# nomadoor/ComfyUI-Video-Stabilizer

Hardware: AMD Instinct MI355X
Metric: stabilized frames/sec (1080p, similarity mode) (higher is better)
Workload: dtype f32; 1 GPU; C2: 256-frame clip, 1920x1080, Video Stabilizer Flow (DIS) similarity + crop_and_pad, defaults (strength 0.7, smooth 0.5, 16 fps), device-resident in/out, entered at the node's input adaptation; frames_per_gpu=256, total_frames=256

## Files before the change

### comfyui-video-stabilizer_amd/csrc/vstab_dis.hip

```cpp
#include "vstab_internal.h"
#include <cstdlib>
#include <cfloat>
#include <algorithm>
#include <cmath>
#include <memory>

namespace {

constexpr float DIS_EPS = 0.001f;
constexpr float DIS_INF = 1e10f;
constexpr int DIS_BORDER = 16;
constexpr int PSZ = 8;
constexpr int PSTR = 4;
constexpr int DEFAULT_FINEST = 2;
constexpr int GD_ITERS = 25;
constexpr int VAR_ITERS = 5;
constexpr int SOR_ITERS = 5;
constexpr int MAX_LEVELS = 16;

struct LevelGeom {
    int w, h, ws, hs;
};

unsigned grid_for(long long items, int block = 256)
// ... 141 lines not shown
        const AreaTaps& ax = s_x[x];
        const AreaTaps& ay = s_y[ry];
        float sum = 0.f;
        for (int j = 0; j < ay.n; j++) {
            const uint8_t* row = S + (size_t)(ay.first + j) * sw + ax.first;
            float buf = 0.f;
            for (int k = 0; k < ax.n; k++) buf += row[k] * ax.a[k];
            const float term = ay.a[j] * buf;
            sum = (j == 0) ? term : sum + term;
        }
        D[t] = (uint8_t)sat_u8_round(sum);
    }
}

constexpr int TAIL_MAX_LEVELS = 8;
#ifdef VSTAB_FUSED_TRACE
#define TAIL_MARK(i) do { if (prof_) { const long long now_ = wall_clock64(); a.dbg[i] += now_ - tprev_; tprev_ = now_; } } while (0)
#else
#define TAIL_MARK(i)
#endif
struct TailLevel { uint8_t* dst; int h, w, mode, kx, ky; double scale_x, scale_y; };
struct TailArgs {
#ifdef VSTAB_FUSED_TRACE
    long long* dbg;
#endif
    const uint8_t* src;
    int n, h0, w0, levels;
    TailLevel lv[TAIL_MAX_LEVELS];
    uint8_t* prep_ext;
    short* prep_ix;
    short* prep_iy;
    float* prep_tensor;
    int prep_ws, prep_hs, prep_lds_off;
};

__global__ __launch_bounds__(1024) void pyramid_tail_kernel(TailArgs a)
{
    extern __shared__ __attribute__((aligned(16))) unsigned char tail_lds[];
    const int f = blockIdx.x;
#ifdef VSTAB_FUSED_TRACE
    long long tprev_ = wall_clock64();
    const bool prof_ = a.dbg && blockIdx.x == 7 && threadIdx.x == 0;
#endif
    const int cap0 = (a.h0 * a.w0 + 15) & ~15;
    const int cap1 = (a.lv[0].h * a.lv[0].w + 15) & ~15;
    unsigned char* bufA = tail_lds;
    unsigned char* bufB = tail_lds + cap0;
    AreaTaps* s_x = reinterpret_cast<AreaTaps*>(tail_lds + cap0 + cap1);
    AreaTaps* s_y = s_x + a.lv[0].w;
    {
        const uint8_t* S = a.src + (size_t)f * a.h0 * a.w0;
        const int npx = a.h0 * a.w0;
        if ((reinterpret_cast<uintptr_t>(S) & 3) == 0 && (npx & 3) == 0) {
            const unsigned* s4 = reinterpret_cast<const unsigned*>(S);
            unsigned* d4 = reinterpret_cast<unsigned*>(bufA);
            for (int k = threadIdx.x; k < npx / 4; k += blockDim.x) d4[k] = s4[k];
        } else {
            for (int k = threadIdx.x; k < npx; k += blockDim.x) bufA[k] = S[k];
        }
    }
    __syncthreads();
    TAIL_MARK(0);
    int sh = a.h0, sw = a.w0;
    unsigned char* cur = bufA;
    unsigned char* nxt = bufB;
    for (int l = 0; l < a.levels; l++) {
        const TailLevel& L = a.lv[l];
        const int dh = L.h, dw = L.w;
        if (L.mode == 2) {
            for (int x = threadIdx.x; x < dw; x += blockDim.x) area_taps(x, sw, L.scale_x, s_x[x]);
            for (int y = threadIdx.x; y < dh; y += blockDim.x) area_taps(y, sh, L.scale_y, s_y[y]);
            __syncthreads();
        }
        uint8_t* D = L.dst + (size_t)f * dh * dw;
        if (L.mode == 2 && L.kx <= 4 && L.ky <= 4 && dw <= (int)blockDim.x) {
            const int rows_par = (int)blockDim.x / dw;
            const int x = (int)threadIdx.x % dw, ry = (int)threadIdx.x / dw;
            if (ry < rows_par) {
                const AreaTaps ax = s_x[x];
                const int x0 = ax.first;
                for (int y = ry; y < dh; y += rows_par) {
                    const AreaTaps& ay = s_y[y];
// ... 1122 lines not shown
            Ixs[i] = c.take<short>(px);
            Iys[i] = c.take<short>(px);
            tensor[i] = c.take<float>(5 * (size_t)n * G[i].hs * G[i].ws);
            Ul[i] = c.take<float>((size_t)P * G[i].h * G[i].w);
            Vl[i] = c.take<float>((size_t)P * G[i].h * G[i].w);
        }
        aux = c.take<float>(5 * (size_t)n * F.h * F.ws);
        aux_c = c.take<float>(5 * (size_t)n * G[coarsest].h * G[coarsest].ws);
        Sx = c.take<float>((size_t)P * F.hs * F.ws);
        Sy = c.take<float>((size_t)P * F.hs * F.ws);
        vb.avg = c.take<float>(npF); vb.Iz = c.take<float>(npF);
        vb.D0 = c.take<f4_t>(npF); vb.D1 = c.take<f4_t>(npF);
        vb.UV = c.take<f2_t>(npF); vb.dA = c.take<f2_t>(npF); vb.dB = c.take<f2_t>(npF);
    };
    {
        Carver sizer(nullptr);
        layout(sizer);
        if (ctx->d_dis.reserve(sizer.off + 256)) return 1;
    }
    Carver carver(ctx->d_dis.ptr);
    layout(carver);

    static const bool two_streams = [] { const char* e = getenv("VSTAB_DIS_PREP_STREAM"); return !(e && atoi(e) == 0); }();
    static_assert(sizeof(ctx->ev_prep) / sizeof(ctx->ev_prep[0]) >= MAX_LEVELS, "one event per pyramid level");
    hipStream_t ps = st;
    if (two_streams) {
        VSTAB_HIP(ctx->prep_stream.ensure());
        VSTAB_HIP(ctx->ev_pyramid.ensure());
        for (auto& ev : ctx->ev_prep) VSTAB_HIP(ev.ensure());
        ps = ctx->prep_stream;
    }
    auto prep_timer = std::make_unique<KernelTimer>(ctx, "dis_prep", KernelTimer::DETAIL);
    bool coarsest_prepared = false;
    {
        if (launch_area(st, gray, I[FINEST], n, h, w, G[FINEST].h, G[FINEST].w)) return 1;
        static const bool tail_on = [] { const char* e = getenv("VSTAB_DIS_PYRAMID_TAIL"); return !(e && atoi(e) == 0); }();
        const int tail_levels = coarsest - FINEST;
        size_t tail_lds = 0;
        if (tail_levels >= 1) {
            const LevelGeom& a0 = G[FINEST];
            const LevelGeom& a1 = G[FINEST + 1];
            tail_lds = (((size_t)a0.h * a0.w + 15) & ~size_t(15)) + (((size_t)a1.h * a1.w + 15) & ~size_t(15)) +
                       sizeof(AreaTaps) * ((size_t)a1.w + a1.h);
        }
        if (tail_on && tail_levels >= 1 && tail_levels <= TAIL_MAX_LEVELS && tail_lds <= 150 * 1024) {
            TailArgs ta{};
#ifdef VSTAB_FUSED_TRACE
            ta.dbg = g_dis_dbg ? g_dis_dbg + 16 * 7 : nullptr;
#endif
            {
                const LevelGeom& c = G[coarsest];
                const size_t off = (tail_lds + 15) & ~size_t(15);
                const size_t need = (((size_t)4 * c.h * c.w + 15) & ~size_t(15)) + sizeof(float) * 5 * (size_t)c.h * c.ws;
                if (off + need <= 150 * 1024) {
                    ta.prep_ext = Iext[coarsest]; ta.prep_ix = Ixs[coarsest]; ta.prep_iy = Iys[coarsest]; ta.prep_tensor = tensor[coarsest];
                    ta.prep_ws = c.ws; ta.prep_hs = c.hs; ta.prep_lds_off = (int)off;
                    tail_lds = off + need;
                    coarsest_prepared = true;
                }
            }
            ta.src = I[FINEST]; ta.n = n; ta.h0 = G[FINEST].h; ta.w0 = G[FINEST].w; ta.levels = tail_levels;
            for (int i = FINEST + 1; i <= coarsest; i++) {
                AreaPlan pl;
                if (int rc = plan_area(G[i - 1].h, G[i - 1].w, G[i].h, G[i].w, pl)) return rc;
                TailLevel& tl = ta.lv[i - FINEST - 1];
                tl.dst = I[i]; tl.h = G[i].h; tl.w = G[i].w; tl.mode = pl.mode; tl.kx = pl.isx; tl.ky = pl.isy;
                if (pl.mode == 2) {
                    tl.kx = (int)std::floor(pl.scale_x) + 2; tl.ky = (int)std::floor(pl.scale_y) + 2;
                }
                tl.scale_x = pl.scale_x; tl.scale_y = pl.scale_y;
            }
            if (tail_lds > 64 * 1024)
                VSTAB_HIP(hipFuncSetAttribute(reinterpret_cast<const void*>(pyramid_tail_kernel), hipFuncAttributeMaxDynamicSharedMemorySize, (int)tail_lds));
            hipLaunchKernelGGL(pyramid_tail_kernel, dim3((unsigned)n), dim3(1024), tail_lds, st, ta);
            VSTAB_HIP(hipGetLastError());
        } else {
            for (int i = FINEST + 1; i <= coarsest; i++)
                if (launch_area(st, I[i - 1], I[i], n, G[i - 1].h, G[i - 1].w, G[i].h, G[i].w)) return 1;
        }
    }
    if (two_streams) {
        VSTAB_HIP(hipEventRecord(ctx->ev_pyramid, st));
        VSTAB_HIP(hipStreamWaitEvent(ps, ctx->ev_pyramid, 0));
    }
    for (int i = coarsest; i >= FINEST; i--) {
        const LevelGeom& g = G[i];
        const bool own = i == coarsest;
        if (own && coarsest_prepared) continue;
        hipStream_t s_i = own ? st : ps;
        float* aux_i = own ? aux_c : aux;
        hipLaunchKernelGGL(pad_replicate_kernel, frame_grid((long long)(g.h + 32) * (g.w + 32), n), dim3(256), 0, s_i, I[i], Iext[i], n, g.h, g.w);
        hipLaunchKernelGGL(sobel_kernel, frame_grid((long long)g.h * g.w, n), dim3(256), 0, s_i, I[i], Ixs[i], Iys[i], n, g.h, g.w);
        hipLaunchKernelGGL(tensor_h_kernel, frame_grid((long long)g.h * g.ws, n), dim3(256), 0, s_i, Ixs[i], Iys[i], aux_i, n, g.h, g.w, g.ws);
        hipLaunchKernelGGL(tensor_v_kernel, dim3((unsigned)((g.ws + 63) / 64), (unsigned)n, 5u), dim3(64), 0, s_i, aux_i, tensor[i], n, g.h, g.ws, g.hs);
        VSTAB_HIP(hipGetLastError());
        if (two_streams && !own) VSTAB_HIP(hipEventRecord(ctx->ev_prep[i], ps));
    }
    VSTAB_HIP(hipMemsetAsync(Ul[coarsest], 0, sizeof(float) * (size_t)P * G[coarsest].h * G[coarsest].w, st));
    VSTAB_HIP(hipMemsetAsync(Vl[coarsest], 0, sizeof(float) * (size_t)P * G[coarsest].h * G[coarsest].w, st));

    prep_timer.reset();

    bool grid_fused = false;
    const float zeta = 0.1f, epsilon = 0.001f, alpha = 20.0f, delta = 5.0f, gamma = 10.0f, omega = 1.6f;
    const float zeta2 = zeta * zeta, eps2 = epsilon * epsilon, gamma2 = gamma / 2, delta2 = delta / 2, alpha2 = alpha / 4;

    for (int i = coarsest; i >= FINEST; i--) {
        const LevelGeom& g = G[i];
        PisArgs pa{};
        pa.I = I[i]; pa.Iext = Iext[i]; pa.Ix = Ixs[i]; pa.Iy = Iys[i]; pa.tensor = tensor[i];
        pa.U = Ul[i]; pa.V = Vl[i]; pa.Sx = Sx; pa.Sy = Sy;
        pa.n = n; pa.w = g.w; pa.h = g.h; pa.ws = g.ws; pa.hs = g.hs;
        pa.stripe_sz = (int)std::ceil(g.hs / 8.0);
        pa.spin_limit = 1 << 22;
#ifdef VSTAB_TEST_HOOKS
        if (const char* e = getenv("VSTAB_DEBUG_PIS_SPIN_LIMIT")) pa.spin_limit = atoi(e);
#endif
        pa.status = ctx->status.dev<int>();
        if (two_streams && i != coarsest) VSTAB_HIP(hipStreamWaitEvent(st, ctx->ev_prep[i], 0));
        const size_t lds_bytes = (((size_t)(g.w + 32) * (g.h + 32) + 15) & ~size_t(15)) + sizeof(float) * 2 * (size_t)g.hs * g.ws + sizeof(int) * 2 * (size_t)g.hs;
        VSTAB_REQUIRE(lds_bytes <= 160 * 1024, "vstab_dis_flow_batch: level %dx%d needs %zu B of LDS (> 160 KB)", g.w, g.h, lds_bytes);
        char kind_pis[24], kind_level[24];
        snprintf(kind_pis, sizeof(kind_pis), "dis_pis4_L%d", i);
        snprintf(kind_level, sizeof(kind_level), "dis_level_L%d", i);
        auto stage_timer = std::make_unique<KernelTimer>(ctx, kind_pis, KernelTimer::DETAIL);
        if (pa.stripe_sz > 4) {
            if (lds_bytes > 64 * 1024)
                VSTAB_HIP(hipFuncSetAttribute(reinterpret_cast<const void*>(pis4_kernel<2>), hipFuncAttributeMaxDynamicSharedMemorySize, (int)lds_bytes));
            hipLaunchKernelGGL(pis4_kernel<2>, dim3((unsigned)P * 2), dim3(64 * 2 * PIS_STRIPES_PER_BLOCK), lds_bytes, st, pa);
        } else {
            if (lds_bytes > 64 * 1024)
                VSTAB_HIP(hipFuncSetAttribute(reinterpret_cast<const void*>(pis4_kernel<1>), hipFuncAttributeMaxDynamicSharedMemorySize, (int)lds_bytes));
// ... 118 lines not shown
```

### comfyui-video-stabilizer_amd/csrc/vstab_fit.hip

```cpp
#include "vstab_fit_common.h"

namespace {

#ifndef VSTAB_FIT_THREADS
#define VSTAB_FIT_THREADS 512
#endif
constexpr int FIT_THREADS = VSTAB_FIT_THREADS;
constexpr int FIT_WAVES = FIT_THREADS / 64;
static_assert(FIT_THREADS >= 256 && FIT_THREADS % 64 == 0 && FIT_THREADS <= 1024, "radix_select uses 256 histogram bins");
constexpr int RANSAC_BATCH = 16;
constexpr int MAX_SORT = 16384;

struct FitArgs {
    const float* grid_flow;
    int* vmap;
    vstab_fit_record* out;
    int pairs, gh, gw, step, requested_mode;
    const int* counts;
    int cap;
    const uint8_t* blocked;
};

__device__ void identity_record(vstab_fit_record& r, int nv, int total)
{
    for (int i = 0; i < 9; i++) r.matrix[i] = (i % 4 == 0) ? 1.f : 0.f;
    r.confidence = 0.0; r.residual = 0.0; r.accepted = 0; r.computed = 0; r.valid_points = nv; r.total_points = total;
}

__device__ __forceinline__ unsigned sort_key(float v)
{
    const unsigned b = __float_as_uint(v);
    return (b & 0x80000000u) ? ~b : (b | 0x80000000u);
}
__device__ __forceinline__ float key_value(unsigned k)
{
    return __uint_as_float((k & 0x80000000u) ? (k & 0x7fffffffu) : ~k);
}

__device__ unsigned radix_select(const unsigned* keys, int n, int r, int* hist , int* ctl )
{
    unsigned prefix = 0, mask = 0;
    for (int shift = 24; shift >= 0; shift -= 8) {
        if (threadIdx.x < 256) hist[threadIdx.x] = 0;
        __syncthreads();
        for (int k = threadIdx.x; k < n; k += FIT_THREADS) {
            const unsigned key = keys[k];
            if ((key & mask) == prefix) atomicAdd(&hist[(key >> shift) & 255u], 1);
        }
        __syncthreads();
        if (threadIdx.x < 64) {
            const int l = threadIdx.x;
            const int h0 = hist[4 * l], h1 = hist[4 * l + 1], h2 = hist[4 * l + 2], h3 = hist[4 * l + 3];
            const int mine = h0 + h1 + h2 + h3;
            int incl = mine;
#pragma unroll
            for (int d = 1; d < 64; d <<= 1) {
                const int o = __shfl_up(incl, d);
                if (l >= d) incl += o;
            }
            const int excl = incl - mine;
            if (r >= excl && r < incl) {
                int rr = r - excl, b = 4 * l;
                if (rr >= h0) { rr -= h0; b++; if (rr >= h1) { rr -= h1; b++; if (rr >= h2) { rr -= h2; b++; } } }
                ctl[0] = b; ctl[1] = rr;
            }
        }
        __syncthreads();
        prefix |= (unsigned)ctl[0] << shift;
        mask |= 0xffu << shift;
        r = ctl[1];
        __syncthreads();
    }
    return prefix;
}

template <bool MASKED>
__global__ __launch_bounds__(FIT_THREADS) void fit_kernel(FitArgs a)
{
    __shared__ unsigned s_sort[MAX_SORT];
    __shared__ int s_hist[256];
    __shared__ int s_sel[2];
    __shared__ double s_model[RANSAC_BATCH][6];
    __shared__ float s_modelf[RANSAC_BATCH][6];
    __shared__ int s_idx[RANSAC_BATCH][2];
    __shared__ int s_cnt[RANSAC_BATCH];
    __shared__ double s_red[FIT_WAVES];
    __shared__ int s_redi[FIT_WAVES];
    __shared__ int s_scan[FIT_THREADS];
    __shared__ double s_best[6];
    __shared__ int s_ctl[4];
    __shared__ Rng s_rng;

    const int pair = blockIdx.x, tid = threadIdx.x;
    const bool points = a.gw == 0;
    const int scan = points ? a.counts[pair] : a.gh * a.gw;
    const uint8_t* __restrict__ B0 = MASKED ? a.blocked + (size_t)pair * a.cap : nullptr;
    const uint8_t* __restrict__ B1 = MASKED ? B0 + a.cap : nullptr;
    int* __restrict__ vmap = a.vmap + (size_t)pair * a.cap;
    const Samples smp{a.grid_flow + (size_t)pair * a.cap * (points ? 4 : 2), vmap, a.gw, a.step};
    vstab_fit_record* out = a.out + (size_t)pair * 3;

    const int per = (scan + FIT_THREADS - 1) / FIT_THREADS;
    const int g0 = tid * per, g1 = min(g0 + per, scan);
    int local = 0, admitted = 0;
    for (int g = g0; g < g1; g++) {
        float px, py, cx, cy;
        smp.load(g, px, py, cx, cy);
        if (MASKED) {
            const bool adm = (B0[g] | B1[g]) == 0;
            admitted += adm ? 1 : 0;
            local += (adm && isfinite(cx) && isfinite(cy)) ? 1 : 0;
        } else {
            local += (isfinite(cx) && isfinite(cy)) ? 1 : 0;
        }
    }
    int total = scan;
    if (MASKED) total = block_sum<FIT_WAVES>(admitted, s_redi);
    {
        int incl = local;
#pragma unroll
        for (int d = 1; d < 64; d <<= 1) {
            const int o = __shfl_up(incl, d);
            if ((tid & 63) >= d) incl += o;
        }
        if ((tid & 63) == 63) s_redi[tid >> 6] = incl;
        __syncthreads();
        int before = 0;
        for (int i = 0; i < (tid >> 6); i++) before += s_redi[i];
        s_scan[tid] = before + incl - local;
        if (tid == FIT_THREADS - 1) s_sel[0] = before + incl;
    }
    __syncthreads();
    const int nv = s_sel[0];
    {
        int o = s_scan[tid];
        for (int g = g0; g < g1; g++) {
            float px, py, cx, cy;
            smp.load(g, px, py, cx, cy);
            if ((!MASKED || (B0[g] | B1[g]) == 0) && isfinite(cx) && isfinite(cy)) vmap[o++] = g;
        }
    }
    __syncthreads();
    if (tid < 3) identity_record(out[tid], nv, total);
    if (points ? (total < 12 || nv < 8) : nv < 12) return;
    __threadfence_block();
    __syncthreads();

    if (a.requested_mode >= VSTAB_MODE_SIMILARITY && nv >= 3) {
        if (tid == 0) { s_rng.state = ~0ULL; s_ctl[0] = 0; s_ctl[1] = 2000; s_ctl[2] = 0; s_ctl[3] = 0; }
        __syncthreads();
        const float thr = (float)(2.0 * 2.0);
        while (true) {
            if (tid == 0) {
                Rng r = s_rng;
                for (int c = 0; c < RANSAC_BATCH; c++) {
                    const int i0 = rng_uniform(r, 0, nv);
                    int i1;
                    do { i1 = rng_uniform(r, 0, nv); } while (i1 == i0);
                    s_idx[c][0] = i0; s_idx[c][1] = i1;
                }
                s_rng = r;
            }
            __syncthreads();
            if (tid < RANSAC_BATCH) {
                float x1f, y1f, X1f, Y1f, x2f, y2f, X2f, Y2f;
                smp.load(vmap[s_idx[tid][0]], x1f, y1f, X1f, Y1f);
                smp.load(vmap[s_idx[tid][1]], x2f, y2f, X2f, Y2f);
                const double x1 = x1f, y1 = y1f, x2 = x2f, y2 = y2f, X1 = X1f, Y1 = Y1f, X2 = X2f, Y2 = Y2f;
                const double d = 1. / ((x1 - x2) * (x1 - x2) + (y1 - y2) * (y1 - y2));
                const double S0 = d * ((X1 - X2) * (x1 - x2) + (Y1 - Y2) * (y1 - y2));
                const double S1 = d * ((Y1 - Y2) * (x1 - x2) - (X1 - X2) * (y1 - y2));
                const double S2 = d * ((Y1 - Y2) * (x1 * y2 - x2 * y1) - (X1 * y2 - X2 * y1) * (y1 - y2) - (X1 * x2 - X2 * x1) * (x1 - x2));
                const double S3 = d * (-(X1 - X2) * (x1 * y2 - x2 * y1) - (Y1 * x2 - Y2 * x1) * (x1 - x2) - (Y1 * y2 - Y2 * y1) * (y1 - y2));
                const double M[6] = {S0, -S1, S2, S1, S0, S3};
                for (int k = 0; k < 6; k++) { s_model[tid][k] = M[k]; s_modelf[tid][k] = (float)M[k]; }
                s_cnt[tid] = 0;
            }
            __syncthreads();
            ransac_score_batch<RANSAC_BATCH, FIT_THREADS>(smp, nv, thr, s_cnt, [&](int c, float px, float py, float cx, float cy) {
                return affine_err2(s_modelf[c], px, py, cx, cy);
            });
            __syncthreads();
            if (tid == 0) ransac_replay<RANSAC_BATCH, 6, 2, 1>(s_ctl, s_cnt, s_model, s_best, nv, [](int) { return RANSAC_SOLVED; });
            __syncthreads();
            if (s_ctl[0]) break;
        }
        const int maxGood = s_ctl[3];
        if (maxGood > 0) {
            const float Bf[6] = {(float)s_best[0], (float)s_best[1], (float)s_best[2], (float)s_best[3], (float)s_best[4], (float)s_best[5]};
            double sxx = 0, sx = 0, sy = 0, sX = 0, sY = 0, sxX = 0, syX = 0;
            int ninl = 0;
            smp.for_each_valid<FIT_THREADS>(nv, [&](int, float px, float py, float cx, float cy) {
                if (affine_err2(Bf, px, py, cx, cy) <= thr) {
                    const double x = px, y = py, X = cx, Y = cy;
                    sxx += x * x + y * y; sx += x; sy += y; sX += X; sY += Y;
                    sxX += x * X + y * Y; syX += x * Y - y * X;
                    ninl++;
                }
            });
            sxx = block_sum<FIT_WAVES>(sxx, s_red); sx = block_sum<FIT_WAVES>(sx, s_red); sy = block_sum<FIT_WAVES>(sy, s_red);
            sX = block_sum<FIT_WAVES>(sX, s_red); sY = block_sum<FIT_WAVES>(sY, s_red);
            sxX = block_sum<FIT_WAVES>(sxX, s_red); syX = block_sum<FIT_WAVES>(syX, s_red);
            ninl = block_sum<FIT_WAVES>(ninl, s_redi);
            if (tid == 0) {
                double A[4][5] = {{sxx, 0, sx, sy, sxX}, {0, sxx, -sy, sx, syX}, {sx, -sy, (double)ninl, 0, sX}, {sy, sx, 0, (double)ninl, sY}};
                bool ok = true;
                for (int col = 0; col < 4 && ok; col++) {
                    int piv = col;
                    for (int r = col + 1; r < 4; r++) if (fabs(A[r][col]) > fabs(A[piv][col])) piv = r;
                    if (fabs(A[piv][col]) < 1e-300) { ok = false; break; }
                    if (piv != col) for (int k = 0; k < 5; k++) { const double t = A[piv][k]; A[piv][k] = A[col][k]; A[col][k] = t; }
                    for (int r = col + 1; r < 4; r++) {
                        const double f = A[r][col] / A[col][col];
                        for (int k = col; k < 5; k++) A[r][k] -= f * A[col][k];
                    }
                }
                double sol[4] = {s_best[0], s_best[3], s_best[2], s_best[5]};
                if (ok && ninl > 0) {
                    for (int r = 3; r >= 0; r--) {
                        double v = A[r][4];
                        for (int k = r + 1; k < 4; k++) v -= A[r][k] * sol[k];
                        sol[r] = v / A[r][r];
                    }
                }
                s_best[0] = sol[0]; s_best[1] = -sol[1]; s_best[2] = sol[2];
                s_best[3] = sol[1]; s_best[4] = sol[0]; s_best[5] = sol[3];
            }
            __syncthreads();
            const double M0 = s_best[0], M1 = s_best[1], M2 = s_best[2], M3 = s_best[3], M4 = s_best[4], M5 = s_best[5];
            double res = 0;
            smp.for_each_valid<FIT_THREADS>(nv, [&](int, float px, float py, float cx, float cy) {
                const double x = px, y = py;
                res += fabs(x * M0 + y * M1 + M2 - (double)cx) + fabs(x * M3 + y * M4 + M5 - (double)cy);
            });
            res = block_sum<FIT_WAVES>(res, s_red);
            if (tid == 0) {
                vstab_fit_record& r = out[VSTAB_MODE_SIMILARITY];
                r.computed = 1;
                r.confidence = (double)maxGood / (double)nv;
                if (r.confidence >= 0.1) {
                    r.matrix[0] = (float)M0; r.matrix[1] = (float)M1; r.matrix[2] = (float)M2;
                    r.matrix[3] = (float)M3; r.matrix[4] = (float)M4; r.matrix[5] = (float)M5;
                    r.matrix[6] = 0.f; r.matrix[7] = 0.f; r.matrix[8] = 1.f;
                    r.residual = res / (2.0 * nv);
                    r.accepted = 1;
                }
            }
        } else if (tid == 0) {
            out[VSTAB_MODE_SIMILARITY].computed = 1;
        }
        __syncthreads();
    }

    {
        float med[2];
        for (int axis = 0; axis < 2; axis++) {
            smp.for_each_valid<FIT_THREADS>(nv, [&](int k, float px, float py, float cx, float cy) {
                s_sort[k] = sort_key(axis == 0 ? cx - px : cy - py);
            });
            __syncthreads();
            const int mid = nv / 2;
            const unsigned hi = radix_select(s_sort, nv, mid, s_hist, s_sel);
            if (nv & 1) {
                med[axis] = key_value(hi);
            } else {
                int less = 0;
                unsigned below = 0;
                for (int i = tid; i < nv; i += FIT_THREADS) {
                    const unsigned key = s_sort[i];
                    if (key < hi) { less++; below = key > below ? key : below; }
                }
#pragma unroll
                for (int sft = 32; sft > 0; sft >>= 1) {
                    less += __shfl_down(less, sft);
                    const unsigned o = __shfl_down(below, sft);
                    below = o > below ? o : below;
                }
                if ((tid & 63) == 0) { s_redi[tid >> 6] = less; s_hist[tid >> 6] = (int)below; }
                __syncthreads();
                int total_less = 0;
                unsigned mx = 0;
                for (int i = 0; i < FIT_WAVES; i++) { total_less += s_redi[i]; mx = (unsigned)s_hist[i] > mx ? (unsigned)s_hist[i] : mx; }
                const unsigned lo = total_less == mid ? mx : hi;
                med[axis] = (key_value(lo) + key_value(hi)) / 2.0f;
            }
            __syncthreads();
        }
        const float tx = med[0], ty = med[1];
        double res = 0;
        smp.for_each_valid<FIT_THREADS>(nv, [&](int, float px, float py, float cx, float cy) {
            res += (double)__builtin_fabsf((px + tx) - cx) + (double)__builtin_fabsf((py + ty) - cy);
        });
        res = block_sum<FIT_WAVES>(res, s_red);
        if (tid == 0) {
            vstab_fit_record& r = out[VSTAB_MODE_TRANSLATION];
            r.computed = 1; r.accepted = 1;
            r.matrix[2] = tx; r.matrix[5] = ty;
            r.confidence = (double)nv / (double)total;
            r.residual = res / (2.0 * nv);
        }
    }
}

}

int vstab_fit_homography(vstab_ctx* ctx, const float* grid_flow, const int* vmap, int pairs, int gh, int gw, int step,
                         int cap, vstab_fit_record* d_out);

static int run_fit(vstab_ctx* ctx, const float* data, const int* counts, int pairs, int gh, int gw, int step, int cap,
                   int requested_mode, vstab_fit_record* results, const uint8_t* blocked = nullptr)
{
    VSTAB_HIP(hipSetDevice(ctx->device));
    if (ctx->fit_pairs_pending > 0 && ctx->fit_copy_bytes == 0 && ctx->ev_fit_done) VSTAB_HIP(hipEventSynchronize(ctx->ev_fit_done));
    ctx->fit_pairs_pending = 0; ctx->fit_copy_bytes = 0;
    const size_t rec_bytes = sizeof(vstab_fit_record) * (size_t)pairs * 3;
    const size_t map_bytes = sizeof(int) * (size_t)pairs * cap;
    if (ctx->d_fit.reserve(rec_bytes + map_bytes + 512)) return 1;
    if (ctx->h_fit.reserve(rec_bytes)) return 1;
    char* base = static_cast<char*>(ctx->d_fit.ptr);
// ... 100 lines not shown
```

### comfyui-video-stabilizer_amd/csrc/vstab_fit_common.h

```cpp
#pragma once
#include "vstab_internal.h"
#include <cmath>

namespace {

struct Rng { unsigned long long state; };
__device__ __forceinline__ unsigned rng_next(Rng& r)
{
    r.state = (unsigned long long)(unsigned)r.state * 4164903690ULL + (unsigned)(r.state >> 32);
    return (unsigned)r.state;
}
__device__ __forceinline__ int rng_uniform(Rng& r, int a, int b) { return a == b ? a : (int)(rng_next(r) % (unsigned)(b - a) + a); }

__device__ int ransac_update_num_iters(double p, double ep, int modelPoints, int maxIters)
{
    p = p > 0. ? p : 0.; p = p < 1. ? p : 1.;
    ep = ep > 0. ? ep : 0.; ep = ep < 1. ? ep : 1.;
    double num = 1. - p > 2.2250738585072014e-308 ? 1. - p : 2.2250738585072014e-308;
    double denom = 1. - pow(1. - ep, (double)modelPoints);
    if (denom < 2.2250738585072014e-308) return 0;
    num = log(num);
    denom = log(denom);
    return denom >= 0 || -num >= maxIters * (-denom) ? maxIters : (int)__builtin_rint(num / denom);
}

struct Samples {
    const float* F;
    const int* vmap;
    int gw, step;

    __device__ __forceinline__ void load(int g, float& px, float& py, float& cx, float& cy) const
    {
        if (gw == 0) {
            const float4 v = *reinterpret_cast<const float4*>(F + (size_t)g * 4);
            px = v.x; py = v.y; cx = v.z; cy = v.w;
            return;
        }
        const int gy = g / gw, gx = g - gy * gw;
        px = (float)(gx * step);
        py = (float)(gy * step);
        cx = px + F[(size_t)g * 2];
        cy = py + F[(size_t)g * 2 + 1];
    }

    template <int NT, typename Body>
    __device__ __forceinline__ void for_each_valid(int nv, Body&& body) const
    {
        for (int k = threadIdx.x; k < nv; k += NT) {
            float px, py, cx, cy;
            load(vmap[k], px, py, cx, cy);
            body(k, px, py, cx, cy);
        }
    }
};

template <int WAVES, typename T>
__device__ __forceinline__ T block_sum(T v, T* scratch )
{
#pragma unroll
    for (int s = 32; s > 0; s >>= 1) v += __shfl_down(v, s);
    __syncthreads();
    if ((threadIdx.x & 63) == 0) scratch[threadIdx.x >> 6] = v;
    __syncthreads();
    T total = scratch[0];
#pragma unroll
    for (int i = 1; i < WAVES; i++) total += scratch[i];
    __syncthreads();
    return total;
}

__device__ __forceinline__ float affine_err2(const float* M, float px, float py, float cx, float cy)
{
    const float ea = M[0] * px + M[1] * py + M[2] - cx;
    const float eb = M[3] * px + M[4] * py + M[5] - cy;
    return ea * ea + eb * eb;
}
__device__ __forceinline__ float reproj_err2(const float* H, float px, float py, float cx, float cy)
{
    const float ww = 1.f / (H[6] * px + H[7] * py + 1.f);
    const float ex = (H[0] * px + H[1] * py + H[2]) * ww - cx;
    const float ey = (H[3] * px + H[4] * py + H[5]) * ww - cy;
    return ex * ex + ey * ey;
}

template <int BATCH, int NT, typename Err>
__device__ __forceinline__ void ransac_score_batch(const Samples& samples, int nv, float thr, int* s_cnt, Err&& err)
{
    int cnt[BATCH];
#pragma unroll
    for (int c = 0; c < BATCH; c++) cnt[c] = 0;
    samples.for_each_valid<NT>(nv, [&](int, float px, float py, float cx, float cy) {
#pragma unroll
        for (int c = 0; c < BATCH; c++) cnt[c] += (err(c, px, py, cx, cy) <= thr) ? 1 : 0;
    });
#pragma unroll
    for (int c = 0; c < BATCH; c++) {
        int v = cnt[c];
#pragma unroll
        for (int s = 32; s > 0; s >>= 1) v += __shfl_down(v, s);
        if ((threadIdx.x & 63) == 0 && v) atomicAdd(&s_cnt[c], v);
    }
// ... 26 lines not shown
```

### comfyui-video-stabilizer_amd/csrc/vstab_homography.hip

```cpp
#include "vstab_fit_common.h"

#define VSTAB_HAVE_HOMOGRAPHY 1

namespace {

constexpr int HT = 256;
constexpr int HBATCH = 16;
constexpr int HWAVES = HT / 64;

struct JacWs {
    double A[81];
    double V[81];
    double W[9];
    int indR[9], indC[9];
    double norm[8];
    int go, pad_;
    double pad;
};

__device__ __forceinline__ void group_sync()
{
    __builtin_amdgcn_fence(__ATOMIC_ACQ_REL, "wavefront");
    __builtin_amdgcn_wave_barrier();
}
// ... 146 lines not shown
            for (int k = j; k < 9; k++) LtL[j * 9 + k] += Lx[j] * Lx[k] + Ly[j] * Ly[k];
    }
    ws.norm[0] = cmx; ws.norm[1] = cmy; ws.norm[2] = cMx; ws.norm[3] = cMy;
    ws.norm[4] = smx; ws.norm[5] = smy; ws.norm[6] = sMx; ws.norm[7] = sMy;
    return true;
}

__device__ bool collinear(const float* p, int count)
{
    const int i = count - 1;
    for (int j = 0; j < i; j++) {
        double dx1 = p[j * 2] - p[i * 2], dy1 = p[j * 2 + 1] - p[i * 2 + 1];
        for (int k = 0; k < j; k++) {
            double dx2 = p[k * 2] - p[i * 2], dy2 = p[k * 2 + 1] - p[i * 2 + 1];
            if (fabs(dx2 * dy1 - dy2 * dx1) <= 1.1920928955078125e-07 * (fabs(dx1) + fabs(dy1) + fabs(dx2) + fabs(dy2))) return true;
        }
    }
    return false;
}
__device__ double det3pts(const float* p, int t0, int t1, int t2)
{
    const double a0 = p[t0 * 2], a1 = p[t0 * 2 + 1], a3 = p[t1 * 2], a4 = p[t1 * 2 + 1], a6 = p[t2 * 2], a7 = p[t2 * 2 + 1];
    return a0 * (a4 * 1. - 1. * a7) - a1 * (a3 * 1. - 1. * a6) + 1. * (a3 * a7 - a4 * a6);
}
__device__ bool check_subset(const float* ms1, const float* ms2)
{
    if (collinear(ms1, 4) || collinear(ms2, 4)) return false;
    const int tt[4][3] = {{0, 1, 2}, {1, 2, 3}, {0, 2, 3}, {0, 1, 3}};
    int negative = 0;
    for (int i = 0; i < 4; i++) negative += det3pts(ms1, tt[i][0], tt[i][1], tt[i][2]) * det3pts(ms2, tt[i][0], tt[i][1], tt[i][2]) < 0;
    return negative == 0 || negative == 4;
}

template <int N>
__device__ __forceinline__ void block_sum_many(const double (&acc)[N], double* part, double* out)
{
    const int wave = threadIdx.x >> 6, lane = threadIdx.x & 63;
#pragma unroll
    for (int i = 0; i < N; i++) {
        double v = acc[i];
#pragma unroll
        for (int s = 32; s > 0; s >>= 1) v += __shfl_down(v, s);
        if (lane == 0) part[wave * N + i] = v;
    }
    __syncthreads();
    for (int i = threadIdx.x; i < N; i += HT) out[i] = ((part[i] + part[N + i]) + part[2 * N + i]) + part[3 * N + i];
    __syncthreads();
}

__device__ bool solve_sym(double (*A)[9] , const double* A_in, const double* b, int n, double* x)
{
    for (int r = 0; r < n; r++) {
        for (int c = 0; c < n; c++) A[r][c] = A_in[r * n + c];
        A[r][n] = b[r];
    }
    for (int col = 0; col < n; col++) {
        int piv = col;
        for (int r = col + 1; r < n; r++) if (fabs(A[r][col]) > fabs(A[piv][col])) piv = r;
        if (fabs(A[piv][col]) < 1e-300) return false;
        if (piv != col) for (int k = 0; k <= n; k++) { const double t = A[piv][k]; A[piv][k] = A[col][k]; A[col][k] = t; }
        for (int r = col + 1; r < n; r++) {
            const double f = A[r][col] / A[col][col];
            for (int k = col; k <= n; k++) A[r][k] -= f * A[col][k];
        }
    }
    for (int r = n - 1; r >= 0; r--) {
        double v = A[r][n];
        for (int k = r + 1; k < n; k++) v -= A[r][k] * x[k];
        x[r] = v / A[r][r];
    }
    return true;
}

#ifdef VSTAB_HOMOGRAPHY_TRACE
static long long* g_h_dbg = nullptr;
extern "C" void vstab_homography_dbg(long long* p) { g_h_dbg = p; }
#define H_MARK(i) do { if (prof_) { const long long now_ = wall_clock64(); a.dbg[i] += now_ - tprev_; tprev_ = now_; } } while (0)
#else
#define H_MARK(i)
#endif

struct HArgs {
// ... 11 lines not shown
                                bool want_jac, double* JtJ , double* Jtr , double* rinf, double* s_red, double* s_part ,
                                double* s_sum )
{
    double acc[45];
    for (int i = 0; i < 45; i++) acc[i] = 0;
    double S = 0, rmax = 0;
    samples.for_each_valid<HT>(nv, [&](int, float px, float py, float cx, float cy) {
        if (!(reproj_err2(Hbf, px, py, cx, cy) <= thr)) return;
        const double Mx = px, My = py;
        double w = h[6] * Mx + h[7] * My + 1.;
        w = fabs(w) > 2.220446049250313e-16 ? 1. / w : 0;
        const double xi = (h[0] * Mx + h[1] * My + h[2]) * w;
        const double yi = (h[3] * Mx + h[4] * My + h[5]) * w;
        const double r0 = xi - (double)cx, r1 = yi - (double)cy;
        S += r0 * r0 + r1 * r1;
        rmax = fmax(rmax, fmax(fabs(r0), fabs(r1)));
        if (want_jac) {
            const double J0[8] = {Mx * w, My * w, w, 0, 0, 0, -Mx * w * xi, -My * w * xi};
            const double J1[8] = {0, 0, 0, Mx * w, My * w, w, -Mx * w * yi, -My * w * yi};
            int idx = 0;
            for (int p = 0; p < 8; p++)
                for (int q = p; q < 8; q++) acc[idx++] += J0[p] * J0[q] + J1[p] * J1[q];
            for (int p = 0; p < 8; p++) acc[36 + p] += J0[p] * r0 + J1[p] * r1;
        }
    });
    S = block_sum<HWAVES>(S, s_red);
    for (int s = 32; s > 0; s >>= 1) rmax = fmax(rmax, __shfl_down(rmax, s));
    __syncthreads();
    if ((threadIdx.x & 63) == 0) s_red[threadIdx.x >> 6] = rmax;
    __syncthreads();
    *rinf = fmax(fmax(s_red[0], s_red[1]), fmax(s_red[2], s_red[3]));
    __syncthreads();
    if (want_jac) {
        block_sum_many<45>(acc, s_part, s_sum);
        if (threadIdx.x < 44) {
            const int i = threadIdx.x;
            if (i < 36) {
                int p = 0, base = 0;
                while (i >= base + (8 - p)) { base += 8 - p; p++; }
                const int q = p + (i - base);
                JtJ[p * 8 + q] = s_sum[i]; JtJ[q * 8 + p] = s_sum[i];
            } else {
                Jtr[i - 36] = s_sum[i];
            }
        }
        __syncthreads();
    }
    return S;
}

__global__ __launch_bounds__(HT) void homography_kernel(HArgs a)
{
    __shared__ double s_model[HBATCH][9];
    __shared__ float s_modelf[HBATCH][8];
    __shared__ int s_ok[HBATCH];
    __shared__ int s_idx[HBATCH][4];
    __shared__ int s_cnt[HBATCH];
    __shared__ double s_red[8];
    __shared__ double s_part[4 * 45], s_sum[45];
    __shared__ int s_redi[8];
    __shared__ double s_best[9];
    __shared__ double s_A[64], s_v[8], s_x[8], s_d[8];
    __shared__ double s_lm[8];
    __shared__ int s_ctl[5];
    __shared__ Rng s_rng;
    __shared__ JacWs s_ws[HBATCH];
    double (*elim)[9] = reinterpret_cast<double (*)[9]>(s_ws[1].A);
// ... 93 lines not shown
    double c0 = 0, c1 = 0, c2 = 0, c3 = 0;
    int ninl = 0;
    smp.for_each_valid<HT>(nv, [&](int, float px, float py, float cx, float cy) {
        if (reproj_err2(Hbf, px, py, cx, cy) <= thr) { c0 += cx; c1 += cy; c2 += px; c3 += py; ninl++; }
    });
    double cmx = block_sum<HWAVES>(c0, s_red), cmy = block_sum<HWAVES>(c1, s_red);
    double cMx = block_sum<HWAVES>(c2, s_red), cMy = block_sum<HWAVES>(c3, s_red);
    ninl = block_sum<HWAVES>(ninl, s_redi);
    cmx /= ninl; cmy /= ninl; cMx /= ninl; cMy /= ninl;
    c0 = c1 = c2 = c3 = 0;
    smp.for_each_valid<HT>(nv, [&](int, float px, float py, float cx, float cy) {
        if (reproj_err2(Hbf, px, py, cx, cy) <= thr) { c0 += fabs(cx - cmx); c1 += fabs(cy - cmy); c2 += fabs(px - cMx); c3 += fabs(py - cMy); }
    });
    double smx = block_sum<HWAVES>(c0, s_red), smy = block_sum<HWAVES>(c1, s_red);
    double sMx = block_sum<HWAVES>(c2, s_red), sMy = block_sum<HWAVES>(c3, s_red);
    const double deps = 2.220446049250313e-16;
    const bool degenerate = fabs(smx) < deps || fabs(smy) < deps || fabs(sMx) < deps || fabs(sMy) < deps;
    if (!degenerate) {
        smx = ninl / smx; smy = ninl / smy; sMx = ninl / sMx; sMy = ninl / sMy;
        double acc[45];
        for (int i = 0; i < 45; i++) acc[i] = 0;
        smp.for_each_valid<HT>(nv, [&](int, float px, float py, float cx, float cy) {
            if (!(reproj_err2(Hbf, px, py, cx, cy) <= thr)) return;
            const double x = (cx - cmx) * smx, y = (cy - cmy) * smy;
            const double X = (px - cMx) * sMx, Y = (py - cMy) * sMy;
            const double Lx[9] = {X, Y, 1, 0, 0, 0, -x * X, -x * Y, -x};
            const double Ly[9] = {0, 0, 0, X, Y, 1, -y * X, -y * Y, -y};
            int idx = 0;
            for (int j = 0; j < 9; j++)
                for (int q = j; q < 9; q++) acc[idx++] += Lx[j] * Lx[q] + Ly[j] * Ly[q];
        });
        H_MARK(4);
        double* s_LtL = s_ws[0].A;
        block_sum_many<45>(acc, s_part, s_sum);
        if (tid < 45) {
            int j = 0, base = 0;
            while (tid >= base + (9 - j)) { base += 9 - j; j++; }
            s_LtL[j * 9 + j + (tid - base)] = s_sum[tid];
        }
        __syncthreads();
        H_MARK(5);
        if (tid < 16) {
            if (tid == 0) {
                double* nm = s_ws[0].norm;
                nm[0] = cmx; nm[1] = cmy; nm[2] = cMx; nm[3] = cMy; nm[4] = smx; nm[5] = smy; nm[6] = sMx; nm[7] = sMy;
            }
            group_sync();
            double H[9];
            homography_from_ltl_g16(s_ws[0], tid, H);
            if (tid == 0) for (int i = 0; i < 9; i++) s_best[i] = H[i];
        }
        __syncthreads();
    }
    H_MARK(6);
    double x[8];
    for (int i = 0; i < 8; i++) x[i] = s_best[i];
    double rinf;
    double S = lm_accumulate(smp, nv, Hbf, thr, x, true, s_A, s_v, &rinf, s_red, s_part, s_sum);
    __shared__ double s_D[8];
    if (tid == 0) { for (int i = 0; i < 8; i++) s_D[i] = s_A[i * 8 + i]; s_lm[0] = 1.0; s_lm[1] = 0.75; }
    __syncthreads();
    const double Rlo = 0.25, Rhi = 0.75;
    H_MARK(7);
    for (int iter = 0; iter < 10; iter++) {
        if (tid == 0) {
            double Ap[64];
            for (int i = 0; i < 64; i++) Ap[i] = s_A[i];
// ... 95 lines not shown
```

Measured before the change: 33150 frames/s.

## Fold flow zeroing into pyramid kernel and batch fit reductions and medians

Zeroes the coarsest-level flow inside the pyramid tail kernel instead of issuing two memsets. In the fit kernel it skips building the valid-index map when all samples are valid, walking the grid directly. It also computes both axis medians in one radix-select pass and merges eight separate block reductions into one multi-value reduction. The aim is fewer launches, barriers and indirect loads, at the cost of more shared memory and more complex code paths.

```diff
diff --git a/comfyui-video-stabilizer_amd/csrc/vstab_dis.hip b/comfyui-video-stabilizer_amd/csrc/vstab_dis.hip
--- a/comfyui-video-stabilizer_amd/csrc/vstab_dis.hip
+++ b/comfyui-video-stabilizer_amd/csrc/vstab_dis.hip
@@ -197,6 +197,9 @@
     short* prep_iy;
     float* prep_tensor;
     int prep_ws, prep_hs, prep_lds_off;
+    float* zero_u;
+    float* zero_v;
+    int zero_pairs, zero_count;
 };
 
 __global__ __launch_bounds__(1024) void pyramid_tail_kernel(TailArgs a)
@@ -213,6 +216,11 @@
     unsigned char* bufB = tail_lds + cap0;
     AreaTaps* s_x = reinterpret_cast<AreaTaps*>(tail_lds + cap0 + cap1);
     AreaTaps* s_y = s_x + a.lv[0].w;
+    if (a.zero_u != nullptr && f < a.zero_pairs) {
+        float* u = a.zero_u + (size_t)f * a.zero_count;
+        float* v = a.zero_v + (size_t)f * a.zero_count;
+        for (int k = threadIdx.x; k < a.zero_count; k += blockDim.x) { u[k] = 0.f; v[k] = 0.f; }
+    }
     {
         const uint8_t* S = a.src + (size_t)f * a.h0 * a.w0;
         const int npx = a.h0 * a.w0;
@@ -1401,6 +1409,7 @@
     }
     auto prep_timer = std::make_unique<KernelTimer>(ctx, "dis_prep", KernelTimer::DETAIL);
     bool coarsest_prepared = false;
+    bool start_flow_cleared = false;
     {
         if (launch_area(st, gray, I[FINEST], n, h, w, G[FINEST].h, G[FINEST].w)) return 1;
         static const bool tail_on = [] { const char* e = getenv("VSTAB_DIS_PYRAMID_TAIL"); return !(e && atoi(e) == 0); }();
@@ -1429,6 +1438,8 @@
                 }
             }
             ta.src = I[FINEST]; ta.n = n; ta.h0 = G[FINEST].h; ta.w0 = G[FINEST].w; ta.levels = tail_levels;
+            ta.zero_u = Ul[coarsest]; ta.zero_v = Vl[coarsest]; ta.zero_pairs = P; ta.zero_count = G[coarsest].h * G[coarsest].w;
+            start_flow_cleared = true;
             for (int i = FINEST + 1; i <= coarsest; i++) {
                 AreaPlan pl;
                 if (int rc = plan_area(G[i - 1].h, G[i - 1].w, G[i].h, G[i].w, pl)) return rc;
@@ -1465,8 +1476,10 @@
         VSTAB_HIP(hipGetLastError());
         if (two_streams && !own) VSTAB_HIP(hipEventRecord(ctx->ev_prep[i], ps));
     }
-    VSTAB_HIP(hipMemsetAsync(Ul[coarsest], 0, sizeof(float) * (size_t)P * G[coarsest].h * G[coarsest].w, st));
-    VSTAB_HIP(hipMemsetAsync(Vl[coarsest], 0, sizeof(float) * (size_t)P * G[coarsest].h * G[coarsest].w, st));
+    if (!start_flow_cleared) {
+        VSTAB_HIP(hipMemsetAsync(Ul[coarsest], 0, sizeof(float) * (size_t)P * G[coarsest].h * G[coarsest].w, st));
+        VSTAB_HIP(hipMemsetAsync(Vl[coarsest], 0, sizeof(float) * (size_t)P * G[coarsest].h * G[coarsest].w, st));
+    }
 
     prep_timer.reset();
 
diff --git a/comfyui-video-stabilizer_amd/csrc/vstab_fit.hip b/comfyui-video-stabilizer_amd/csrc/vstab_fit.hip
--- a/comfyui-video-stabilizer_amd/csrc/vstab_fit.hip
+++ b/comfyui-video-stabilizer_amd/csrc/vstab_fit.hip
@@ -37,20 +37,29 @@
     return __uint_as_float((k & 0x80000000u) ? (k & 0x7fffffffu) : ~k);
 }
 
-__device__ unsigned radix_select(const unsigned* keys, int n, int r, int* hist , int* ctl )
-{
-    unsigned prefix = 0, mask = 0;
+template <int AXES>
+__device__ void radix_select(const unsigned* keys, int n, int r, int* hist , int* ctl , unsigned (&sel)[AXES])
+{
+    unsigned prefix[AXES], mask = 0;
+    int rank[AXES];
+#pragma unroll
+    for (int a = 0; a < AXES; a++) { prefix[a] = 0; rank[a] = r; }
     for (int shift = 24; shift >= 0; shift -= 8) {
-        if (threadIdx.x < 256) hist[threadIdx.x] = 0;
+        for (int i = threadIdx.x; i < 256 * AXES; i += FIT_THREADS) hist[i] = 0;
         __syncthreads();
         for (int k = threadIdx.x; k < n; k += FIT_THREADS) {
-            const unsigned key = keys[k];
-            if ((key & mask) == prefix) atomicAdd(&hist[(key >> shift) & 255u], 1);
-        }
-        __syncthreads();
-        if (threadIdx.x < 64) {
-            const int l = threadIdx.x;
-            const int h0 = hist[4 * l], h1 = hist[4 * l + 1], h2 = hist[4 * l + 2], h3 = hist[4 * l + 3];
+#pragma unroll
+            for (int a = 0; a < AXES; a++) {
+                const unsigned key = keys[a * n + k];
+                if ((key & mask) == prefix[a]) atomicAdd(&hist[256 * a + ((key >> shift) & 255u)], 1);
+            }
+        }
+        __syncthreads();
+        if (threadIdx.x < 64 * AXES) {
+            const int ax = threadIdx.x >> 6, l = threadIdx.x & 63;
+            const int* h = hist + 256 * ax;
+            const int want = ax ? rank[AXES - 1] : rank[0];
+            const int h0 = h[4 * l], h1 = h[4 * l + 1], h2 = h[4 * l + 2], h3 = h[4 * l + 3];
             const int mine = h0 + h1 + h2 + h3;
             int incl = mine;
 #pragma unroll
@@ -59,33 +68,85 @@
                 if (l >= d) incl += o;
             }
             const int excl = incl - mine;
-            if (r >= excl && r < incl) {
-                int rr = r - excl, b = 4 * l;
+            if (want >= excl && want < incl) {
+                int rr = want - excl, b = 4 * l;
                 if (rr >= h0) { rr -= h0; b++; if (rr >= h1) { rr -= h1; b++; if (rr >= h2) { rr -= h2; b++; } } }
-                ctl[0] = b; ctl[1] = rr;
-            }
-        }
-        __syncthreads();
-        prefix |= (unsigned)ctl[0] << shift;
+                ctl[2 * ax] = b; ctl[2 * ax + 1] = rr;
+            }
+        }
+        __syncthreads();
+#pragma unroll
+        for (int a = 0; a < AXES; a++) {
+            prefix[a] |= (unsigned)ctl[2 * a] << shift;
+            rank[a] = ctl[2 * a + 1];
+        }
         mask |= 0xffu << shift;
-        r = ctl[1];
-        __syncthreads();
-    }
-    return prefix;
+        __syncthreads();
+    }
+#pragma unroll
+    for (int a = 0; a < AXES; a++) sel[a] = prefix[a];
+}
+
+template <int AXES>
+__device__ void medians(const unsigned* keys, int nv, int* hist, int* ctl, int* redi, float (&med)[AXES])
+{
+    const int tid = threadIdx.x, mid = nv / 2;
+    unsigned hi[AXES];
+    radix_select<AXES>(keys, nv, mid, hist, ctl, hi);
+    if (nv & 1) {
+#pragma unroll
+        for (int a = 0; a < AXES; a++) med[a] = key_value(hi[a]);
+    } else {
+        int less[AXES];
+        unsigned below[AXES];
+#pragma unroll
+        for (int a = 0; a < AXES; a++) { less[a] = 0; below[a] = 0; }
+        for (int i = tid; i < nv; i += FIT_THREADS) {
+#pragma unroll
+            for (int a = 0; a < AXES; a++) {
+                const unsigned key = keys[a * nv + i];
+                if (key < hi[a]) { less[a]++; below[a] = key > below[a] ? key : below[a]; }
+            }
+        }
+#pragma unroll
+        for (int a = 0; a < AXES; a++) {
+#pragma unroll
+            for (int sft = 32; sft > 0; sft >>= 1) {
+                less[a] += __shfl_down(less[a], sft);
+                const unsigned o = __shfl_down(below[a], sft);
+                below[a] = o > below[a] ? o : below[a];
+            }
+            if ((tid & 63) == 0) { redi[a * FIT_WAVES + (tid >> 6)] = less[a]; hist[a * FIT_WAVES + (tid >> 6)] = (int)below[a]; }
+        }
+        __syncthreads();
+#pragma unroll
+        for (int a = 0; a < AXES; a++) {
+            int total_less = 0;
+            unsigned mx = 0;
+            for (int i = 0; i < FIT_WAVES; i++) {
+                total_less += redi[a * FIT_WAVES + i];
+                mx = (unsigned)hist[a * FIT_WAVES + i] > mx ? (unsigned)hist[a * FIT_WAVES + i] : mx;
+            }
+            const unsigned lo = total_less == mid ? mx : hi[a];
+            med[a] = (key_value(lo) + key_value(hi[a])) / 2.0f;
+        }
+    }
+    __syncthreads();
 }
 
 template <bool MASKED>
 __global__ __launch_bounds__(FIT_THREADS) void fit_kernel(FitArgs a)
 {
     __shared__ unsigned s_sort[MAX_SORT];
-    __shared__ int s_hist[256];
-    __shared__ int s_sel[2];
+    __shared__ int s_hist[512];
+    __shared__ int s_sel[4];
     __shared__ double s_model[RANSAC_BATCH][6];
     __shared__ float s_modelf[RANSAC_BATCH][6];
     __shared__ int s_idx[RANSAC_BATCH][2];
     __shared__ int s_cnt[RANSAC_BATCH];
     __shared__ double s_red[FIT_WAVES];
-    __shared__ int s_redi[FIT_WAVES];
+    __shared__ double s_part[FIT_WAVES * 8], s_sum[8];
+    __shared__ int s_redi[2 * FIT_WAVES];
     __shared__ int s_scan[FIT_THREADS];
     __shared__ double s_best[6];
     __shared__ int s_ctl[4];
@@ -97,23 +158,34 @@
     const uint8_t* __restrict__ B0 = MASKED ? a.blocked + (size_t)pair * a.cap : nullptr;
     const uint8_t* __restrict__ B1 = MASKED ? B0 + a.cap : nullptr;
     int* __restrict__ vmap = a.vmap + (size_t)pair * a.cap;
-    const Samples smp{a.grid_flow + (size_t)pair * a.cap * (points ? 4 : 2), vmap, a.gw, a.step};
+    const float* __restrict__ F = a.grid_flow + (size_t)pair * a.cap * (points ? 4 : 2);
     vstab_fit_record* out = a.out + (size_t)pair * 3;
 
     const int per = (scan + FIT_THREADS - 1) / FIT_THREADS;
     const int g0 = tid * per, g1 = min(g0 + per, scan);
-    int local = 0, admitted = 0;
-    for (int g = g0; g < g1; g++) {
-        float px, py, cx, cy;
-        smp.load(g, px, py, cx, cy);
-        if (MASKED) {
-            const bool adm = (B0[g] | B1[g]) == 0;
-            admitted += adm ? 1 : 0;
-            local += (adm && isfinite(cx) && isfinite(cy)) ? 1 : 0;
-        } else {
-            local += (isfinite(cx) && isfinite(cy)) ? 1 : 0;
-        }
-    }
+    int admitted = 0;
+    auto scan_range = [&](bool count_admitted, auto&& body) {
+        int gy = points ? 0 : g0 / a.gw, gx = points ? 0 : g0 - gy * a.gw;
+        for (int g = g0; g < g1; g++) {
+            float cx, cy;
+            if (points) {
+                const float4 v = *reinterpret_cast<const float4*>(F + (size_t)g * 4);
+                cx = v.z; cy = v.w;
+            } else {
+                cx = (float)(gx * a.step) + F[(size_t)g * 2];
+                cy = (float)(gy * a.step) + F[(size_t)g * 2 + 1];
+                if (++gx == a.gw) { gx = 0; gy++; }
+            }
+            bool adm = true;
+            if (MASKED) {
+                adm = (B0[g] | B1[g]) == 0;
+                if (count_admitted) admitted += adm ? 1 : 0;
+            }
+            body(g, adm && isfinite(cx) && isfinite(cy));
+        }
+    };
+    int local = 0;
+    scan_range(true, [&](int, bool ok) { local += ok ? 1 : 0; });
     int total = scan;
     if (MASKED) total = block_sum<FIT_WAVES>(admitted, s_redi);
     {
@@ -132,13 +204,11 @@
     }
     __syncthreads();
     const int nv = s_sel[0];
-    {
+    const bool dense = nv == scan;
+    const Samples smp{F, vmap, a.gw, a.step, dense};
+    if (!dense || a.requested_mode >= VSTAB_MODE_PERSPECTIVE) {
         int o = s_scan[tid];
-        for (int g = g0; g < g1; g++) {
-            float px, py, cx, cy;
-            smp.load(g, px, py, cx, cy);
-            if ((!MASKED || (B0[g] | B1[g]) == 0) && isfinite(cx) && isfinite(cy)) vmap[o++] = g;
-        }
+        scan_range(false, [&](int g, bool ok) { if (ok) vmap[o++] = g; });
     }
     __syncthreads();
     if (tid < 3) identity_record(out[tid], nv, total);
@@ -164,8 +234,8 @@
             __syncthreads();
             if (tid < RANSAC_BATCH) {
                 float x1f, y1f, X1f, Y1f, x2f, y2f, X2f, Y2f;
-                smp.load(vmap[s_idx[tid][0]], x1f, y1f, X1f, Y1f);
-                smp.load(vmap[s_idx[tid][1]], x2f, y2f, X2f, Y2f);
+                smp.load(smp.entry(s_idx[tid][0]), x1f, y1f, X1f, Y1f);
+                smp.load(smp.entry(s_idx[tid][1]), x2f, y2f, X2f, Y2f);
                 const double x1 = x1f, y1 = y1f, x2 = x2f, y2 = y2f, X1 = X1f, Y1 = Y1f, X2 = X2f, Y2 = Y2f;
                 const double d = 1. / ((x1 - x2) * (x1 - x2) + (y1 - y2) * (y1 - y2));
                 const double S0 = d * ((X1 - X2) * (x1 - x2) + (Y1 - Y2) * (y1 - y2));
@@ -198,10 +268,12 @@
                     ninl++;
                 }
             });
-            sxx = block_sum<FIT_WAVES>(sxx, s_red); sx = block_sum<FIT_WAVES>(sx, s_red); sy = block_sum<FIT_WAVES>(sy, s_red);
-            sX = block_sum<FIT_WAVES>(sX, s_red); sY = block_sum<FIT_WAVES>(sY, s_red);
-            sxX = block_sum<FIT_WAVES>(sxX, s_red); syX = block_sum<FIT_WAVES>(syX, s_red);
-            ninl = block_sum<FIT_WAVES>(ninl, s_redi);
+            {
+                const double acc[8] = {sxx, sx, sy, sX, sY, sxX, syX, (double)ninl};
+                block_sum_many<FIT_WAVES, 8>(acc, s_part, s_sum);
+                sxx = s_sum[0]; sx = s_sum[1]; sy = s_sum[2]; sX = s_sum[3]; sY = s_sum[4]; sxX = s_sum[5]; syX = s_sum[6];
+                ninl = (int)s_sum[7];
+            }
             if (tid == 0) {
                 double A[4][5] = {{sxx, 0, sx, sy, sxX}, {0, sxx, -sy, sx, syX}, {sx, -sy, (double)ninl, 0, sX}, {sy, sx, 0, (double)ninl, sY}};
                 bool ok = true;
@@ -254,37 +326,23 @@
 
     {
         float med[2];
-        for (int axis = 0; axis < 2; axis++) {
+        if (2 * nv <= MAX_SORT) {
             smp.for_each_valid<FIT_THREADS>(nv, [&](int k, float px, float py, float cx, float cy) {
-                s_sort[k] = sort_key(axis == 0 ? cx - px : cy - py);
+                s_sort[k] = sort_key(cx - px);
+                s_sort[nv + k] = sort_key(cy - py);
             });
             __syncthreads();
-            const int mid = nv / 2;
-            const unsigned hi = radix_select(s_sort, nv, mid, s_hist, s_sel);
-            if (nv & 1) {
-                med[axis] = key_value(hi);
-            } else {
-                int less = 0;
-                unsigned below = 0;
-                for (int i = tid; i < nv; i += FIT_THREADS) {
-                    const unsigned key = s_sort[i];
-                    if (key < hi) { less++; below = key > below ? key : below; }
-                }
-#pragma unroll
-                for (int sft = 32; sft > 0; sft >>= 1) {
-                    less += __shfl_down(less, sft);
-                    const unsigned o = __shfl_down(below, sft);
-                    below = o > below ? o : below;
-                }
-                if ((tid & 63) == 0) { s_redi[tid >> 6] = less; s_hist[tid >> 6] = (int)below; }
+            medians<2>(s_sort, nv, s_hist, s_sel, s_redi, med);
+        } else {
+            for (int axis = 0; axis < 2; axis++) {
+                smp.for_each_valid<FIT_THREADS>(nv, [&](int k, float px, float py, float cx, float cy) {
+                    s_sort[k] = sort_key(axis == 0 ? cx - px : cy - py);
+                });
                 __syncthreads();
-                int total_less = 0;
-                unsigned mx = 0;
-                for (int i = 0; i < FIT_WAVES; i++) { total_less += s_redi[i]; mx = (unsigned)s_hist[i] > mx ? (unsigned)s_hist[i] : mx; }
-                const unsigned lo = total_less == mid ? mx : hi;
-                med[axis] = (key_value(lo) + key_value(hi)) / 2.0f;
-            }
-            __syncthreads();
+                float m[1];
+                medians<1>(s_sort, nv, s_hist, s_sel, s_redi, m);
+                med[axis] = m[0];
+            }
         }
         const float tx = med[0], ty = med[1];
         double res = 0;
diff --git a/comfyui-video-stabilizer_amd/csrc/vstab_fit_common.h b/comfyui-video-stabilizer_amd/csrc/vstab_fit_common.h
--- a/comfyui-video-stabilizer_amd/csrc/vstab_fit_common.h
+++ b/comfyui-video-stabilizer_amd/csrc/vstab_fit_common.h
@@ -28,6 +28,9 @@
     const float* F;
     const int* vmap;
     int gw, step;
+    bool dense = false;
+
+    __device__ __forceinline__ int entry(int k) const { return dense ? k : vmap[k]; }
 
     __device__ __forceinline__ void load(int g, float& px, float& py, float& cx, float& cy) const
     {
@@ -46,9 +49,24 @@
     template <int NT, typename Body>
     __device__ __forceinline__ void for_each_valid(int nv, Body&& body) const
     {
+        const bool walk = dense && gw > 0;
+        int dx = 0, dy = 0, gx = 0, gy = 0;
+        if (walk) {
+            dy = NT / gw; dx = NT - dy * gw;
+            gy = (int)threadIdx.x / gw; gx = (int)threadIdx.x - gy * gw;
+        }
         for (int k = threadIdx.x; k < nv; k += NT) {
             float px, py, cx, cy;
-            load(vmap[k], px, py, cx, cy);
+            if (walk) {
+                px = (float)(gx * step);
+                py = (float)(gy * step);
+                cx = px + F[(size_t)k * 2];
+                cy = py + F[(size_t)k * 2 + 1];
+                gx += dx; gy += dy;
+                if (gx >= gw) { gx -= gw; gy++; }
+            } else {
+                load(entry(k), px, py, cx, cy);
+            }
             body(k, px, py, cx, cy);
         }
     }
@@ -67,6 +85,27 @@
     for (int i = 1; i < WAVES; i++) total += scratch[i];
     __syncthreads();
     return total;
+}
+
+template <int WAVES, int N>
+__device__ __forceinline__ void block_sum_many(const double (&acc)[N], double* part, double* out)
+{
+    const int wave = threadIdx.x >> 6, lane = threadIdx.x & 63;
+#pragma unroll
+    for (int i = 0; i < N; i++) {
+        double v = acc[i];
+#pragma unroll
+        for (int s = 32; s > 0; s >>= 1) v += __shfl_down(v, s);
+        if (lane == 0) part[wave * N + i] = v;
+    }
+    __syncthreads();
+    for (int i = threadIdx.x; i < N; i += WAVES * 64) {
+        double total = part[i];
+#pragma unroll
+        for (int w = 1; w < WAVES; w++) total += part[w * N + i];
+        out[i] = total;
+    }
+    __syncthreads();
 }
 
 __device__ __forceinline__ float affine_err2(const float* M, float px, float py, float cx, float cy)
diff --git a/comfyui-video-stabilizer_amd/csrc/vstab_homography.hip b/comfyui-video-stabilizer_amd/csrc/vstab_homography.hip
--- a/comfyui-video-stabilizer_amd/csrc/vstab_homography.hip
+++ b/comfyui-video-stabilizer_amd/csrc/vstab_homography.hip
@@ -202,22 +202,6 @@
     return negative == 0 || negative == 4;
 }
 
-template <int N>
-__device__ __forceinline__ void block_sum_many(const double (&acc)[N], double* part, double* out)
-{
-    const int wave = threadIdx.x >> 6, lane = threadIdx.x & 63;
-#pragma unroll
-    for (int i = 0; i < N; i++) {
-        double v = acc[i];
-#pragma unroll
-        for (int s = 32; s > 0; s >>= 1) v += __shfl_down(v, s);
-        if (lane == 0) part[wave * N + i] = v;
-    }
-    __syncthreads();
-    for (int i = threadIdx.x; i < N; i += HT) out[i] = ((part[i] + part[N + i]) + part[2 * N + i]) + part[3 * N + i];
-    __syncthreads();
-}
-
 __device__ bool solve_sym(double (*A)[9] , const double* A_in, const double* b, int n, double* x)
 {
     for (int r = 0; r < n; r++) {
@@ -295,7 +279,7 @@
     *rinf = fmax(fmax(s_red[0], s_red[1]), fmax(s_red[2], s_red[3]));
     __syncthreads();
     if (want_jac) {
-        block_sum_many<45>(acc, s_part, s_sum);
+        block_sum_many<HWAVES, 45>(acc, s_part, s_sum);
         if (threadIdx.x < 44) {
             const int i = threadIdx.x;
             if (i < 36) {
@@ -455,7 +439,7 @@
         });
         H_MARK(4);
         double* s_LtL = s_ws[0].A;
-        block_sum_many<45>(acc, s_part, s_sum);
+        block_sum_many<HWAVES, 45>(acc, s_part, s_sum);
         if (tid < 45) {
             int j = 0, base = 0;
             while (tid >= base + (9 - j)) { base += 9 - j; j++; }
```

Result: no change. 33420 frames/s (median of 6 runs) (+0.8%).
